# Zehong-Ma/MagCache

Measured on NVIDIA H100. Metric: denoising_steps_per_sec, higher is better.
Workload: dtype bf16

## Files before the change

### magcache_b200/csrc/attn_wgmma.cu

```cuda
#include <cstdlib>

#include "common.cuh"
#include "ptx.cuh"
#include "tma_host.cuh"

#ifndef MC_ATTN_EMU_DEFAULT
#define MC_ATTN_EMU_DEFAULT 0
#endif

namespace mc {

constexpr int kHD = 128;
constexpr int kLongMinLk = 1024;

struct AttnParams {
  int Lq, Lk, heads;
  int q_blocks, full_units, tail_units, tail_split;
  float* part_o;
  float2* part_ml;
  float scale_log2;
  __nv_bfloat16* out;
  int64_t ldo;
  int tile_rot;
  const uint32_t* seg_flags;
  const uint32_t* seg_epoch;
  int seg_rows;
};

struct WorkItem {
  int q_block, head;
  int split, nsplit;
  int tail_unit;
};

__device__ __forceinline__ WorkItem work_item(const AttnParams& p) {
  WorkItem w;
  int c = blockIdx.x, unit;
  if (c < p.full_units) {
    unit = c, w.split = 0, w.nsplit = 1, w.tail_unit = 0;
  } else {
    c -= p.full_units;
    w.tail_unit = c / p.tail_split;
    w.split = c - w.tail_unit * p.tail_split;
    w.nsplit = p.tail_split;
    unit = p.full_units + w.tail_unit;
  }
  w.head = unit / p.q_blocks;
  w.q_block = unit - w.head * p.q_blocks;
  return w;
}

template <uint32_t EMU_MASK>
__device__ __forceinline__ float exp2_sel(float x, int group) {
  return ((EMU_MASK >> (group & 7)) & 1u) ? ptx::ex2_emul(x) : ptx::ex2_approx(x);
}

__device__ __forceinline__ void wait_segments(const AttnParams& p, int row0, int rows) {
  if (p.seg_flags == nullptr) return;
  const uint32_t want = *reinterpret_cast<const volatile uint32_t*>(p.seg_epoch);
  const int last = min(row0 + rows, p.Lk) - 1;
  const int s0 = row0 / p.seg_rows, s1 = last / p.seg_rows;
  for (int s = s0; s <= s1; ++s) {
    const uint32_t* f = p.seg_flags + s;
    const long long t0 = clock64();
    for (;;) {
      uint32_t v;
      asm volatile("ld.acquire.sys.global.u32 %0, [%1];" : "=r"(v) : "l"(f) : "memory");
      if (static_cast<int32_t>(v - want) >= 0) break;
      __nanosleep(100);
      if (clock64() - t0 > MC_MBAR_TIMEOUT_CYCLES) {
        MC_DIAG("attention: key segment %d never arrived (flag %u, epoch %u)\n", s, v, want);
        __trap();
      }
    }
  }
  asm volatile("fence.proxy.async;" ::: "memory");
}

namespace ak {
constexpr int kBQ = 128;
constexpr int kQBytes = kBQ * kHD * 2;
constexpr int kThreads = 384;
constexpr int kProducerRegs = 24, kConsumerRegs = 240;
template <int BKV>
struct Layout {
  static constexpr int kKBytes = BKV * kHD * 2;
  static constexpr int kVBytes = BKV * kHD * 2;
  static constexpr int kOffK = kQBytes;
  static constexpr int kOffV = kOffK + 2 * kKBytes;
  static constexpr int kOffBar = kOffV + 2 * kVBytes;
  static constexpr int kSmem = kOffBar + 128;
};
}

template <int BKV, uint32_t EMU_MASK>
__global__ void __launch_bounds__(ak::kThreads, 1)
    attn_kernel(const __grid_constant__ CUtensorMap tmap_q, const __grid_constant__ CUtensorMap tmap_k,
                const __grid_constant__ CUtensorMap tmap_v, const AttnParams p) {
  using namespace ak;
  using L = Layout<BKV>;
  extern __shared__ __align__(1024) uint8_t smem[];
  uint64_t* bars = reinterpret_cast<uint64_t*>(smem + L::kOffBar);
  uint64_t* q_full = bars + 0;
  uint64_t* k_full = bars + 1;
  uint64_t* k_empty = bars + 3;
  uint64_t* v_full = bars + 5;
  uint64_t* v_empty = bars + 7;

  const int warp = threadIdx.x >> 5, lane = threadIdx.x & 31;
  const WorkItem wi = work_item(p);
  const int q0 = wi.q_block * kBQ;
  const int head = wi.head;
  const int total_tiles = (p.Lk + BKV - 1) / BKV;
  const int per_split = (total_tiles + wi.nsplit - 1) / wi.nsplit;
  const int t0 = wi.split * per_split;
  const int n_tiles = min(per_split, total_tiles - t0);
  auto tile_of = [&](int j) {
    int t = p.tile_rot + t0 + j;
    return t >= total_tiles ? t - total_tiles : t;
  };

  if (threadIdx.x == 0) {
    if ((ptx::smem_u32(smem) & 1023u) != 0) {
      MC_DIAG("attn_kernel: dynamic smem base not 1024-aligned\n");
      __trap();
    }
    ptx::prefetch_tmap(&tmap_q);
    ptx::prefetch_tmap(&tmap_k);
    ptx::prefetch_tmap(&tmap_v);
    ptx::mbar_init(q_full, 1);
    for (int s = 0; s < 2; ++s) {
      ptx::mbar_init(&k_full[s], 1);
      ptx::mbar_init(&k_empty[s], 8);
      ptx::mbar_init(&v_full[s], 1);
      ptx::mbar_init(&v_empty[s], 8);
    }
    ptx::fence_mbar_init();
  }
  __syncthreads();

  if (warp < 4) {
    ptx::setmaxnreg_dec<kProducerRegs>();
    if (warp == 0) {
      if (ptx::elect_one()) {
        ptx::mbar_expect_tx(q_full, kQBytes);
        ptx::tma_load_2d(smem, &tmap_q, q_full, head * kHD, q0);
        ptx::tma_load_2d(smem + kQBytes / 2, &tmap_q, q_full, head * kHD + 64, q0);
      }
      __syncwarp();
      for (int j = 0; j < n_tiles; ++j) {
        const int s = j & 1;
        const uint32_t ph = (j >> 1) & 1;
        const int kv0 = tile_of(j) * BKV;
        if (p.seg_flags != nullptr) {
          if (lane == 0) wait_segments(p, kv0, BKV);
          __syncwarp();
        }
        ptx::mbar_wait(&k_empty[s], ph ^ 1);
        if (ptx::elect_one()) {
          ptx::mbar_expect_tx(&k_full[s], L::kKBytes);
          ptx::tma_load_2d(smem + L::kOffK + s * L::kKBytes, &tmap_k, &k_full[s], head * kHD, kv0);
          ptx::tma_load_2d(smem + L::kOffK + s * L::kKBytes + L::kKBytes / 2, &tmap_k, &k_full[s], head * kHD + 64, kv0);
        }
        __syncwarp();
        ptx::mbar_wait(&v_empty[s], ph ^ 1);
        if (ptx::elect_one()) {
          ptx::mbar_expect_tx(&v_full[s], L::kVBytes);
          ptx::tma_load_2d(smem + L::kOffV + s * L::kVBytes, &tmap_v, &v_full[s], head * kHD, kv0);
          ptx::tma_load_2d(smem + L::kOffV + s * L::kVBytes + L::kVBytes / 2, &tmap_v, &v_full[s], head * kHD + 64, kv0);
        }
        __syncwarp();
      }
    }
  } else {
    ptx::setmaxnreg_inc<kConsumerRegs>();
    const int wg = (warp >> 2) - 1;
    const int r = wg * 64 + (warp & 3) * 16 + (lane >> 2);
    const int cq = 2 * (lane & 3);
    const uint32_t q_base = ptx::smem_u32(smem) + wg * (64 * 128);
    const uint32_t k_base = ptx::smem_u32(smem + L::kOffK), v_base = ptx::smem_u32(smem + L::kOffV);
    int j_ragged = -1;
    if (p.Lk % BKV != 0) {
      int jr = total_tiles - 1 - p.tile_rot - t0;
      if (jr < 0) jr += total_tiles;
      if (jr < n_tiles) j_ragged = jr;
    }
    float o[kHD / 2];
#pragma unroll
    for (int i = 0; i < kHD / 2; ++i) o[i] = 0.f;
    float m0 = -INFINITY, m1 = -INFINITY, l0 = 0.f, l1 = 0.f;
    bool timed_out = false;
    ptx::mbar_wait_or_flag(q_full, 0, timed_out);

    constexpr uint32_t kTurnThreads = 256;
    const uint32_t bar_own = 1 + wg, bar_other = 2 - wg;
    auto turn_begin = [&] { ptx::named_bar_sync(bar_own, kTurnThreads); };
    auto turn_end = [&] { ptx::named_bar_arrive(bar_other, kTurnThreads); };
    if (wg == 0) ptx::named_bar_arrive(bar_own, kTurnThreads);

    float sc[BKV / 2];
    uint32_t pa[BKV / 16][4];
    const int valid = p.Lk - (total_tiles - 1) * BKV;
    auto issue_s = [&](int j) {
      const int s = j & 1;
      ptx::wgmma_fence();
#pragma unroll
      for (int kk = 0; kk < kHD / 16; ++kk) {
        const uint64_t da = ptx::gmma_desc_sw128_kmajor(q_base + (kk >> 2) * (kQBytes / 2)) + 2 * (kk & 3);
        const uint64_t db = ptx::gmma_desc_sw128_kmajor(k_base + s * L::kKBytes + (kk >> 2) * (L::kKBytes / 2)) + 2 * (kk & 3);
        if constexpr (BKV == 128) {
          ptx::wgmma_m64n128k16_ss(sc, da, db, kk != 0 ? 1u : 0u);
        } else {
          ptx::wgmma_m64n64k16_ss(sc, da, db, kk != 0 ? 1u : 0u);
        }
      }
      ptx::wgmma_commit();
    };
    auto issue_pv = [&](int j) {
      const int s = j & 1;
      ptx::fence_regs(o);
      ptx::wgmma_fence();
      const uint64_t dv = ptx::gmma_desc_sw128_mnmajor(v_base + s * L::kVBytes, BKV * 128);
#pragma unroll
      for (int kk = 0; kk < BKV / 16; ++kk)
        ptx::wgmma_m64n128k16_rs_tb(o, pa[kk], dv + static_cast<uint64_t>(kk * (2048 / 16)), 1u);
      ptx::wgmma_commit();
    };
    auto softmax = [&](int j, float& f0, float& f1) {
      ptx::fence_regs(sc);
      __syncwarp();
      if (lane == 0) ptx::mbar_arrive(&k_empty[j & 1]);
      if (j == j_ragged) {
#pragma unroll
        for (int i = 0; i < BKV / 8; ++i)
#pragma unroll
          for (int e = 0; e < 4; ++e)
            if (8 * i + cq + (e & 1) >= valid) sc[4 * i + e] = -INFINITY;
      }
      float mx0 = -INFINITY, mx1 = -INFINITY;
#pragma unroll
      for (int i = 0; i < BKV / 8; ++i) {
        mx0 = fmaxf(mx0, fmaxf(sc[4 * i], sc[4 * i + 1]));
        mx1 = fmaxf(mx1, fmaxf(sc[4 * i + 2], sc[4 * i + 3]));
      }
#pragma unroll
      for (int off = 1; off <= 2; off <<= 1) {
        mx0 = fmaxf(mx0, __shfl_xor_sync(0xffffffffu, mx0, off));
        mx1 = fmaxf(mx1, __shfl_xor_sync(0xffffffffu, mx1, off));
      }
      const float mn0 = fmaxf(m0, mx0 * p.scale_log2), mn1 = fmaxf(m1, mx1 * p.scale_log2);
      f0 = ptx::ex2_approx(m0 - mn0), f1 = ptx::ex2_approx(m1 - mn1);
      m0 = mn0, m1 = mn1;
      l0 *= f0, l1 *= f1;
#pragma unroll
      for (int i = 0; i < BKV / 8; ++i) {
        sc[4 * i] = exp2_sel<EMU_MASK>(fmaf(sc[4 * i], p.scale_log2, -m0), i);
        sc[4 * i + 1] = exp2_sel<EMU_MASK>(fmaf(sc[4 * i + 1], p.scale_log2, -m0), i);
        sc[4 * i + 2] = exp2_sel<EMU_MASK>(fmaf(sc[4 * i + 2], p.scale_log2, -m1), i);
        sc[4 * i + 3] = exp2_sel<EMU_MASK>(fmaf(sc[4 * i + 3], p.scale_log2, -m1), i);
        l0 += sc[4 * i] + sc[4 * i + 1];
        l1 += sc[4 * i + 2] + sc[4 * i + 3];
      }
    };
    auto pack_p = [&] {
#pragma unroll
      for (int i = 0; i < BKV / 8; ++i) {
        pa[i >> 1][(i & 1) * 2] = pack_bf16x2(sc[4 * i], sc[4 * i + 1]);
        pa[i >> 1][(i & 1) * 2 + 1] = pack_bf16x2(sc[4 * i + 2], sc[4 * i + 3]);
      }
    };
    auto release_v = [&](int j) {
      ptx::fence_regs(o);
      __syncwarp();
      if (lane == 0) ptx::mbar_arrive(&v_empty[j & 1]);
    };
    auto rescale_o = [&](float f0, float f1) {
#pragma unroll
      for (int i = 0; i < kHD / 8; ++i) {
        o[4 * i] *= f0, o[4 * i + 1] *= f0;
        o[4 * i + 2] *= f1, o[4 * i + 3] *= f1;
      }
    };
    {
      ptx::mbar_wait_or_flag(&k_full[0], 0, timed_out);
      turn_begin();
      issue_s(0);
      turn_end();
      ptx::wgmma_wait<0>();
      float f0, f1;
      softmax(0, f0, f1);
      rescale_o(f0, f1);
      pack_p();
    }
    for (int j = 1; j < n_tiles; ++j) {
      ptx::mbar_wait_or_flag(&k_full[j & 1], (j >> 1) & 1, timed_out);
      ptx::mbar_wait_or_flag(&v_full[(j - 1) & 1], ((j - 1) >> 1) & 1, timed_out);
      turn_begin();
      issue_s(j);
      issue_pv(j - 1);
      turn_end();
      ptx::wgmma_wait<1>();
      float f0, f1;
      softmax(j, f0, f1);
      ptx::wgmma_wait<0>();
      release_v(j - 1);
      rescale_o(f0, f1);
      pack_p();
    }
    {
      const int j = n_tiles - 1;
      ptx::mbar_wait_or_flag(&v_full[j & 1], (j >> 1) & 1, timed_out);
      turn_begin();
      issue_pv(j);
      if (wg == 0) turn_end();
      ptx::wgmma_wait<0>();
      release_v(j);
    }
    if (timed_out) __trap();

#pragma unroll
    for (int off = 1; off <= 2; off <<= 1) {
      l0 += __shfl_xor_sync(0xffffffffu, l0, off);
      l1 += __shfl_xor_sync(0xffffffffu, l1, off);
    }
    const bool partial = wi.nsplit > 1;
#pragma unroll
    for (int h = 0; h < 2; ++h) {
      const float inv_l = 1.0f / (h ? l1 : l0);
      const int rt = r + 8 * h;
      const int row = q0 + rt;
      if (row >= p.Lq) continue;
      if (partial) {
        const int64_t prow = (static_cast<int64_t>(wi.split) * p.tail_units + wi.tail_unit) * kBQ + rt;
        if ((lane & 3) == 0) p.part_ml[prow] = make_float2(h ? m1 : m0, h ? l1 : l0);
        float* dst = p.part_o + prow * kHD + cq;
#pragma unroll
        for (int i = 0; i < kHD / 8; ++i)
          *reinterpret_cast<float2*>(dst + 8 * i) = make_float2(o[4 * i + 2 * h] * inv_l, o[4 * i + 2 * h + 1] * inv_l);
      } else {
        __nv_bfloat16* dst = p.out + static_cast<int64_t>(row) * p.ldo + head * kHD + cq;
#pragma unroll
        for (int i = 0; i < kHD / 8; ++i)
          *reinterpret_cast<uint32_t*>(dst + 8 * i) = pack_bf16x2(o[4 * i + 2 * h] * inv_l, o[4 * i + 2 * h + 1] * inv_l);
      }
    }
  }
}

__global__ void __launch_bounds__(256) attn_combine_kernel(const float* __restrict__ part_o, const float2* __restrict__ part_ml, int nsplit,
                                                           int tail_units, int full_units, int q_blocks, int rows_per_cta, int Lq,
                                                           __nv_bfloat16* __restrict__ out, int64_t ldo) {
  constexpr int kGroups = kHD / 8;
  const int64_t total = static_cast<int64_t>(tail_units) * rows_per_cta * kGroups;
  const int64_t split_stride = static_cast<int64_t>(tail_units) * rows_per_cta;
  for (int64_t i = static_cast<int64_t>(blockIdx.x) * blockDim.x + threadIdx.x; i < total; i += static_cast<int64_t>(gridDim.x) * blockDim.x) {
    const int64_t prow = i / kGroups;
    const int g = static_cast<int>(i - prow * kGroups);
    const int tu = static_cast<int>(prow / rows_per_cta), r = static_cast<int>(prow - static_cast<int64_t>(tu) * rows_per_cta);
    const int unit = full_units + tu;
    const int head = unit / q_blocks, row = (unit - head * q_blocks) * rows_per_cta + r;
    if (row >= Lq) continue;
    float mmax = -INFINITY;
    for (int s = 0; s < nsplit; ++s) mmax = fmaxf(mmax, part_ml[s * split_stride + prow].x);
    float acc[8] = {0.f, 0.f, 0.f, 0.f, 0.f, 0.f, 0.f, 0.f};
    float wsum = 0.f;
    for (int s = 0; s < nsplit; ++s) {
      const float2 ml = part_ml[s * split_stride + prow];
      const float w = ml.y * ptx::ex2_approx(ml.x - mmax);
      wsum += w;
      float v[8];
      ptx::ld_nc_v8_f32(part_o + (s * split_stride + prow) * kHD + g * 8, v);
#pragma unroll
      for (int j = 0; j < 8; ++j) acc[j] = fmaf(w, v[j], acc[j]);
    }
    const float inv = 1.0f / wsum;
#pragma unroll
    for (int j = 0; j < 8; ++j) acc[j] *= inv;
    *reinterpret_cast<uint4*>(out + static_cast<int64_t>(row) * ldo + head * kHD + g * 8) = pack_bf16x8(acc);
  }
}

struct AttnPlan {
  bool long_kernel;
  int q_blocks, kv_tile, total_tiles, rows_per_cta;
  int full_units, tail_units, tail_split;
  size_t ws_bytes;
  int grid() const { return full_units + tail_units * tail_split; }
};

static int env_int(const char* name, int lo, int hi, int dflt) {
  const char* e = getenv(name);
  if (!e || !*e) return dflt;
  const int v = atoi(e);
  return (v < lo || v > hi) ? dflt : v;
}

static AttnPlan plan_attention(int Lq, int Lk, int heads, bool need_long = false) {
  AttnPlan pl;
  const int forced_splits = env_int("MC_ATTN_SPLITS", 1, 16, 0);
  const int kernel_sel = env_int("MC_ATTN_KERNEL", 0, 2, 0);
  pl.long_kernel = need_long || kernel_sel == 2 || (kernel_sel == 0 && Lk >= kLongMinLk);
  pl.rows_per_cta = ak::kBQ;
  pl.kv_tile = pl.long_kernel ? 128 : 64;
  pl.q_blocks = (Lq + pl.rows_per_cta - 1) / pl.rows_per_cta;
  pl.total_tiles = (Lk + pl.kv_tile - 1) / pl.kv_tile;
  const int64_t units = static_cast<int64_t>(pl.q_blocks) * heads;
  const int slots = num_sms();
  const int min_tiles_per_split = pl.long_kernel ? 4 : 8;
  int full = static_cast<int>(units), tail = 0, split = 1;
  if (forced_splits > 0) {
    if (forced_splits > 1) full = 0, tail = static_cast<int>(units), split = forced_splits;
  } else {
    const int rem = static_cast<int>(units % slots);
    const int by_tiles = pl.total_tiles / min_tiles_per_split;
    int f = rem > 0 ? slots / rem : 1;
    if (f > 8) f = 8;
    if (f > by_tiles) f = by_tiles;
    if (f >= 2) full = static_cast<int>(units) - rem, tail = rem, split = f;
  }
  if (split > pl.total_tiles) split = pl.total_tiles;
  if (split > 1) {
    const int per = (pl.total_tiles + split - 1) / split;
    split = (pl.total_tiles + per - 1) / per;
  }
  if (split <= 1) full = static_cast<int>(units), tail = 0, split = 1;
  pl.full_units = full, pl.tail_units = tail, pl.tail_split = split;
  pl.ws_bytes = tail > 0 ? static_cast<size_t>(split) * tail * pl.rows_per_cta * (kHD * sizeof(float) + sizeof(float2)) : 0;
  return pl;
}

}

extern "C" int32_t mc_attn_workspace_bytes(int32_t Lq, int32_t Lk, int32_t heads, int64_t* bytes_out) {
  MC_CHECK_ARG(bytes_out != nullptr && Lq >= 1 && Lk >= 1 && heads >= 1, "mc_attn_workspace_bytes: bad arguments");
  const size_t a = mc::plan_attention(Lq, Lk, heads, false).ws_bytes, b = mc::plan_attention(Lq, Lk, heads, true).ws_bytes;
  *bytes_out = static_cast<int64_t>(a > b ? a : b);
  return MC_OK;
}

extern "C" int32_t mc_attn_fwd_ex(const void* q, int64_t ldq, const void* k, int64_t ldk, const void* v, int64_t ldv, void* out,
                                  int64_t ldo, int32_t Lq, int32_t Lk, int32_t heads, float scale, void* workspace,
                                  int64_t workspace_bytes, int32_t first_key_row, const uint32_t* seg_flags, const uint32_t* seg_epoch,
                                  int32_t seg_rows, void* stream) {
  MC_CHECK_ARG(q && k && v && out, "mc_attn_fwd: null pointer");
  MC_CHECK_ARG(Lq >= 1 && Lk >= 1 && heads >= 1, "mc_attn_fwd: Lq=%d Lk=%d heads=%d", Lq, Lk, heads);
  const int64_t width = static_cast<int64_t>(heads) * mc::kHD;
  MC_CHECK_ARG(ldq >= width && ldk >= width && ldo >= width && ldv >= width, "mc_attn_fwd: leading dimensions too small");
  MC_CHECK_ARG(ldq % 8 == 0 && ldk % 8 == 0 && ldv % 8 == 0 && ldo % 8 == 0, "mc_attn_fwd: leading dimensions must be multiples of 8");
  MC_CHECK_ARG(mc::aligned16(q) && mc::aligned16(k) && mc::aligned16(v) && mc::aligned16(out), "mc_attn_fwd: pointers must be 16-byte aligned");
  MC_CHECK_ARG(first_key_row >= 0 && first_key_row < Lk, "mc_attn_fwd: first_key_row=%d outside [0, %d)", first_key_row, Lk);
  MC_CHECK_ARG(seg_flags == nullptr || (seg_rows >= 1 && seg_epoch != nullptr), "mc_attn_fwd: seg_rows=%d / null epoch", seg_rows);
  const mc::AttnPlan pl = mc::plan_attention(Lq, Lk, heads, first_key_row != 0 || seg_flags != nullptr);
  MC_CHECK_ARG(static_cast<int64_t>(pl.q_blocks) * heads * 8 < INT32_MAX, "mc_attn_fwd: grid too large");
  if (pl.tail_units > 0) {
    MC_CHECK_ARG(workspace != nullptr && workspace_bytes >= static_cast<int64_t>(pl.ws_bytes) && (reinterpret_cast<uintptr_t>(workspace) & 31u) == 0,
                 "mc_attn_fwd: split-KV needs a 32-byte aligned workspace of %lld bytes (mc_attn_workspace_bytes), got %lld",
                 static_cast<long long>(pl.ws_bytes), static_cast<long long>(workspace_bytes));
  }
  const int q_box = mc::ak::kBQ;
  CUtensorMap tq, tk, tv;
  int32_t rc = mc::make_tmap_bf16_2d(&tq, q, static_cast<uint64_t>(Lq), static_cast<uint64_t>(width), static_cast<uint64_t>(ldq), q_box, 64);
  if (rc) return rc;
  rc = mc::make_tmap_bf16_2d(&tk, k, static_cast<uint64_t>(Lk), static_cast<uint64_t>(width), static_cast<uint64_t>(ldk), pl.kv_tile, 64);
  if (rc) return rc;
  rc = mc::make_tmap_bf16_2d(&tv, v, static_cast<uint64_t>(Lk), static_cast<uint64_t>(width), static_cast<uint64_t>(ldv), pl.kv_tile, 64);
  if (rc) return rc;

  float* part_o = static_cast<float*>(workspace);
  const size_t part_rows = static_cast<size_t>(pl.tail_split) * pl.tail_units * pl.rows_per_cta;
  float2* part_ml = pl.tail_units > 0 ? reinterpret_cast<float2*>(part_o + part_rows * mc::kHD) : nullptr;
  mc::AttnParams p{};
  p.Lq = Lq, p.Lk = Lk, p.heads = heads;
  p.q_blocks = pl.q_blocks, p.full_units = pl.full_units, p.tail_units = pl.tail_units, p.tail_split = pl.tail_split;
  p.part_o = pl.tail_units > 0 ? part_o : nullptr, p.part_ml = part_ml;
  p.scale_log2 = scale * 1.4426950408889634f;
  p.out = static_cast<__nv_bfloat16*>(out), p.ldo = ldo;
  p.tile_rot = ((first_key_row + pl.kv_tile - 1) / pl.kv_tile) % pl.total_tiles;
  p.seg_flags = seg_flags, p.seg_epoch = seg_epoch, p.seg_rows = seg_rows > 0 ? seg_rows : Lk;

  dim3 grid(pl.grid(), 1, 1);
  cudaStream_t st = static_cast<cudaStream_t>(stream);
  if (pl.long_kernel) {
    static mc::PerDeviceOnce once[4];
    const int emu = mc::env_int("MC_ATTN_EMU", 0, 4, MC_ATTN_EMU_DEFAULT);
#define MC_LAUNCH_LONG(MASK, IDX)                                                                                                    \
  do {                                                                                                                               \
    rc = mc::set_max_smem_once(mc::attn_kernel<128, MASK>, mc::ak::Layout<128>::kSmem, once[IDX], "cudaFuncSetAttribute(attn smem)"); \
    if (rc) return rc;                                                                                                               \
    mc::attn_kernel<128, MASK><<<grid, mc::ak::kThreads, mc::ak::Layout<128>::kSmem, st>>>(tq, tk, tv, p);                           \
  } while (0)
    switch (emu) {
      case 2: MC_LAUNCH_LONG(0x88u, 1); break;
      case 3: MC_LAUNCH_LONG(0x92u, 2); break;
      case 4: MC_LAUNCH_LONG(0xAAu, 3); break;
      default: MC_LAUNCH_LONG(0x00u, 0); break;
    }
#undef MC_LAUNCH_LONG
  } else {
    static mc::PerDeviceOnce once;
    rc = mc::set_max_smem_once(mc::attn_kernel<64, 0u>, mc::ak::Layout<64>::kSmem, once, "cudaFuncSetAttribute(attn smem)");
    if (rc) return rc;
    mc::attn_kernel<64, 0u><<<grid, mc::ak::kThreads, mc::ak::Layout<64>::kSmem, st>>>(tq, tk, tv, p);
  }
  MC_CHECK_LAUNCH("attn_kernel launch");
  if (pl.tail_units > 0) {
    const int64_t total = static_cast<int64_t>(pl.tail_units) * pl.rows_per_cta * (mc::kHD / 8);
    const int64_t want = (total + 255) / 256, cap = static_cast<int64_t>(mc::num_sms()) * 8;
    mc::attn_combine_kernel<<<static_cast<int>(want < cap ? want : cap), 256, 0, st>>>(
        p.part_o, p.part_ml, pl.tail_split, pl.tail_units, pl.full_units, pl.q_blocks, pl.rows_per_cta, Lq, static_cast<__nv_bfloat16*>(out), ldo);
    MC_CHECK_LAUNCH("attn_combine_kernel launch");
  }
  return MC_OK;
}

extern "C" int32_t mc_attn_fwd(const void* q, int64_t ldq, const void* k, int64_t ldk, const void* v, int64_t ldv, void* out,
                               int64_t ldo, int32_t Lq, int32_t Lk, int32_t heads, float scale, void* workspace,
                               int64_t workspace_bytes, void* stream) {
  return mc_attn_fwd_ex(q, ldq, k, ldk, v, ldv, out, ldo, Lq, Lk, heads, scale, workspace, workspace_bytes, 0, nullptr, nullptr, 0, stream);
}
```

Before: 1.660.

## Multicast K/V tiles across 2-CTA clusters in long attention kernel

For the long (BKV=128) attention kernel, CTAs are grouped into clusters of two that process adjacent query blocks of the same head. Each CTA loads half of every K/V tile and multicasts it to both CTAs, so each tile is read from L2 once per cluster instead of once per CTA. Empty-barrier release now arrives on both CTAs' barriers, work-item mapping and q_blocks are padded to cluster multiples, and slots are sized by the cluster occupancy query. The costs are cross-CTA coupling, where the slower CTA stalls its partner, possible padding of wasted query blocks, and a cluster sync at exit.

```diff
diff --git a/magcache_b200/csrc/attn_wgmma.cu b/magcache_b200/csrc/attn_wgmma.cu
--- a/magcache_b200/csrc/attn_wgmma.cu
+++ b/magcache_b200/csrc/attn_wgmma.cu
@@ -33,6 +33,7 @@
   int tail_unit;
 };
 
+template <int C>
 __device__ __forceinline__ WorkItem work_item(const AttnParams& p) {
   WorkItem w;
   int c = blockIdx.x, unit;
@@ -40,8 +41,9 @@
     unit = c, w.split = 0, w.nsplit = 1, w.tail_unit = 0;
   } else {
     c -= p.full_units;
-    w.tail_unit = c / p.tail_split;
-    w.split = c - w.tail_unit * p.tail_split;
+    const int cl = c / C, tail_cl = cl / p.tail_split;
+    w.split = cl - tail_cl * p.tail_split;
+    w.tail_unit = C * tail_cl + (c - cl * C);
     w.nsplit = p.tail_split;
     unit = p.full_units + w.tail_unit;
   }
@@ -78,19 +80,25 @@
 }
 
 namespace ak {
+template <int BKV>
+constexpr int kCluster = BKV == 128 ? 2 : 1;
+constexpr int kStages = 2;
 constexpr int kBQ = 128;
 constexpr int kQBytes = kBQ * kHD * 2;
 constexpr int kThreads = 384;
+constexpr int kConsumerWarps = 8;
 constexpr int kProducerRegs = 24, kConsumerRegs = 240;
 template <int BKV>
 struct Layout {
   static constexpr int kKBytes = BKV * kHD * 2;
   static constexpr int kVBytes = BKV * kHD * 2;
   static constexpr int kOffK = kQBytes;
-  static constexpr int kOffV = kOffK + 2 * kKBytes;
-  static constexpr int kOffBar = kOffV + 2 * kVBytes;
+  static constexpr int kOffV = kOffK + kStages * kKBytes;
+  static constexpr int kOffBar = kOffV + kStages * kVBytes;
   static constexpr int kSmem = kOffBar + 128;
 };
+__device__ __forceinline__ int stage(int j) { return static_cast<int>(static_cast<uint32_t>(j) % kStages); }
+__device__ __forceinline__ uint32_t phase(int j) { return (static_cast<uint32_t>(j) / kStages) & 1u; }
 }
 
 template <int BKV, uint32_t EMU_MASK>
@@ -99,16 +107,18 @@
                 const __grid_constant__ CUtensorMap tmap_v, const AttnParams p) {
   using namespace ak;
   using L = Layout<BKV>;
+  constexpr int C = kCluster<BKV>;
   extern __shared__ __align__(1024) uint8_t smem[];
   uint64_t* bars = reinterpret_cast<uint64_t*>(smem + L::kOffBar);
   uint64_t* q_full = bars + 0;
   uint64_t* k_full = bars + 1;
-  uint64_t* k_empty = bars + 3;
-  uint64_t* v_full = bars + 5;
-  uint64_t* v_empty = bars + 7;
+  uint64_t* k_empty = bars + 1 + kStages;
+  uint64_t* v_full = bars + 1 + 2 * kStages;
+  uint64_t* v_empty = bars + 1 + 3 * kStages;
 
   const int warp = threadIdx.x >> 5, lane = threadIdx.x & 31;
-  const WorkItem wi = work_item(p);
+  const uint32_t rank = C > 1 ? ptx::cluster_ctarank() : 0u;
+  const WorkItem wi = work_item<C>(p);
   const int q0 = wi.q_block * kBQ;
   const int head = wi.head;
   const int total_tiles = (p.Lk + BKV - 1) / BKV;
@@ -129,15 +139,20 @@
     ptx::prefetch_tmap(&tmap_k);
     ptx::prefetch_tmap(&tmap_v);
     ptx::mbar_init(q_full, 1);
-    for (int s = 0; s < 2; ++s) {
+    for (int s = 0; s < kStages; ++s) {
       ptx::mbar_init(&k_full[s], 1);
-      ptx::mbar_init(&k_empty[s], 8);
+      ptx::mbar_init(&k_empty[s], C * kConsumerWarps);
       ptx::mbar_init(&v_full[s], 1);
-      ptx::mbar_init(&v_empty[s], 8);
+      ptx::mbar_init(&v_empty[s], C * kConsumerWarps);
     }
     ptx::fence_mbar_init();
   }
-  __syncthreads();
+  if constexpr (C > 1) {
+    ptx::cluster_arrive();
+    ptx::cluster_wait();
+  } else {
+    __syncthreads();
+  }
 
   if (warp < 4) {
     ptx::setmaxnreg_dec<kProducerRegs>();
@@ -148,9 +163,19 @@
         ptx::tma_load_2d(smem + kQBytes / 2, &tmap_q, q_full, head * kHD + 64, q0);
       }
       __syncwarp();
+      constexpr uint16_t kAll = (1u << C) - 1;
+      const int col = head * kHD + static_cast<int>(rank) * 64;
+      auto load = [&](uint8_t* dst, const CUtensorMap* tmap, uint64_t* bar, int kv0) {
+        if constexpr (C > 1) {
+          ptx::tma_load_2d_multicast(dst + rank * (L::kKBytes / 2), tmap, bar, col, kv0, kAll);
+        } else {
+          ptx::tma_load_2d(dst, tmap, bar, head * kHD, kv0);
+          ptx::tma_load_2d(dst + L::kKBytes / 2, tmap, bar, head * kHD + 64, kv0);
+        }
+      };
       for (int j = 0; j < n_tiles; ++j) {
-        const int s = j & 1;
-        const uint32_t ph = (j >> 1) & 1;
+        const int s = stage(j);
+        const uint32_t ph = phase(j);
         const int kv0 = tile_of(j) * BKV;
         if (p.seg_flags != nullptr) {
           if (lane == 0) wait_segments(p, kv0, BKV);
@@ -159,15 +184,13 @@
         ptx::mbar_wait(&k_empty[s], ph ^ 1);
         if (ptx::elect_one()) {
           ptx::mbar_expect_tx(&k_full[s], L::kKBytes);
-          ptx::tma_load_2d(smem + L::kOffK + s * L::kKBytes, &tmap_k, &k_full[s], head * kHD, kv0);
-          ptx::tma_load_2d(smem + L::kOffK + s * L::kKBytes + L::kKBytes / 2, &tmap_k, &k_full[s], head * kHD + 64, kv0);
+          load(smem + L::kOffK + s * L::kKBytes, &tmap_k, &k_full[s], kv0);
         }
         __syncwarp();
         ptx::mbar_wait(&v_empty[s], ph ^ 1);
         if (ptx::elect_one()) {
           ptx::mbar_expect_tx(&v_full[s], L::kVBytes);
-          ptx::tma_load_2d(smem + L::kOffV + s * L::kVBytes, &tmap_v, &v_full[s], head * kHD, kv0);
-          ptx::tma_load_2d(smem + L::kOffV + s * L::kVBytes + L::kVBytes / 2, &tmap_v, &v_full[s], head * kHD + 64, kv0);
+          load(smem + L::kOffV + s * L::kVBytes, &tmap_v, &v_full[s], kv0);
         }
         __syncwarp();
       }
@@ -198,11 +221,21 @@
     auto turn_end = [&] { ptx::named_bar_arrive(bar_other, kTurnThreads); };
     if (wg == 0) ptx::named_bar_arrive(bar_own, kTurnThreads);
 
+    auto release = [&](uint64_t* bar) {
+      __syncwarp();
+      if (lane == 0) {
+        if constexpr (C > 1) {
+          for (uint32_t c = 0; c < C; ++c) ptx::mbar_arrive_cluster(bar, c);
+        } else {
+          ptx::mbar_arrive(bar);
+        }
+      }
+    };
     float sc[BKV / 2];
     uint32_t pa[BKV / 16][4];
     const int valid = p.Lk - (total_tiles - 1) * BKV;
     auto issue_s = [&](int j) {
-      const int s = j & 1;
+      const int s = stage(j);
       ptx::wgmma_fence();
 #pragma unroll
       for (int kk = 0; kk < kHD / 16; ++kk) {
@@ -217,7 +250,7 @@
       ptx::wgmma_commit();
     };
     auto issue_pv = [&](int j) {
-      const int s = j & 1;
+      const int s = stage(j);
       ptx::fence_regs(o);
       ptx::wgmma_fence();
       const uint64_t dv = ptx::gmma_desc_sw128_mnmajor(v_base + s * L::kVBytes, BKV * 128);
@@ -228,8 +261,7 @@
     };
     auto softmax = [&](int j, float& f0, float& f1) {
       ptx::fence_regs(sc);
-      __syncwarp();
-      if (lane == 0) ptx::mbar_arrive(&k_empty[j & 1]);
+      release(&k_empty[stage(j)]);
       if (j == j_ragged) {
 #pragma unroll
         for (int i = 0; i < BKV / 8; ++i)
@@ -271,8 +303,7 @@
     };
     auto release_v = [&](int j) {
       ptx::fence_regs(o);
-      __syncwarp();
-      if (lane == 0) ptx::mbar_arrive(&v_empty[j & 1]);
+      release(&v_empty[stage(j)]);
     };
     auto rescale_o = [&](float f0, float f1) {
 #pragma unroll
@@ -293,8 +324,8 @@
       pack_p();
     }
     for (int j = 1; j < n_tiles; ++j) {
-      ptx::mbar_wait_or_flag(&k_full[j & 1], (j >> 1) & 1, timed_out);
-      ptx::mbar_wait_or_flag(&v_full[(j - 1) & 1], ((j - 1) >> 1) & 1, timed_out);
+      ptx::mbar_wait_or_flag(&k_full[stage(j)], phase(j), timed_out);
+      ptx::mbar_wait_or_flag(&v_full[stage(j - 1)], phase(j - 1), timed_out);
       turn_begin();
       issue_s(j);
       issue_pv(j - 1);
@@ -309,7 +340,7 @@
     }
     {
       const int j = n_tiles - 1;
-      ptx::mbar_wait_or_flag(&v_full[j & 1], (j >> 1) & 1, timed_out);
+      ptx::mbar_wait_or_flag(&v_full[stage(j)], phase(j), timed_out);
       turn_begin();
       issue_pv(j);
       if (wg == 0) turn_end();
@@ -344,6 +375,10 @@
           *reinterpret_cast<uint32_t*>(dst + 8 * i) = pack_bf16x2(o[4 * i + 2 * h] * inv_l, o[4 * i + 2 * h + 1] * inv_l);
       }
     }
+  }
+  if constexpr (C > 1) {
+    ptx::cluster_arrive();
+    ptx::cluster_wait();
   }
 }
 
@@ -395,6 +430,42 @@
   return (v < lo || v > hi) ? dflt : v;
 }
 
+template <int BKV>
+struct AttnLaunch {
+  cudaLaunchAttribute attr[1];
+  cudaLaunchConfig_t cfg = {};
+  AttnLaunch(int grid, cudaStream_t st) {
+    attr[0].id = cudaLaunchAttributeClusterDimension;
+    attr[0].val.clusterDim.x = ak::kCluster<BKV>, attr[0].val.clusterDim.y = 1, attr[0].val.clusterDim.z = 1;
+    cfg.gridDim = dim3(grid, 1, 1);
+    cfg.blockDim = dim3(ak::kThreads, 1, 1);
+    cfg.dynamicSmemBytes = ak::Layout<BKV>::kSmem;
+    cfg.stream = st;
+    cfg.attrs = attr;
+    cfg.numAttrs = ak::kCluster<BKV> > 1 ? 1 : 0;
+  }
+};
+
+template <int BKV>
+static int attn_slots() {
+  constexpr int C = ak::kCluster<BKV>;
+  if (C == 1) return num_sms();
+  static int cached[kMaxDevices] = {};
+  const int d = current_device();
+  if (cached[d] > 0) return cached[d];
+  AttnLaunch<BKV> la(C * num_sms(), nullptr);
+  int n = 0;
+  if (cudaFuncSetAttribute(attn_kernel<BKV, 0u>, cudaFuncAttributeMaxDynamicSharedMemorySize, ak::Layout<BKV>::kSmem) != cudaSuccess ||
+      cudaOccupancyMaxActiveClusters(&n, attn_kernel<BKV, 0u>, &la.cfg) != cudaSuccess)
+    n = 0;
+  if (n < 1) {
+    (void)cudaGetLastError();
+    return num_sms() / C * C;
+  }
+  cached[d] = C * n;
+  return cached[d];
+}
+
 static AttnPlan plan_attention(int Lq, int Lk, int heads, bool need_long = false) {
   AttnPlan pl;
   const int forced_splits = env_int("MC_ATTN_SPLITS", 1, 16, 0);
@@ -402,10 +473,12 @@
   pl.long_kernel = need_long || kernel_sel == 2 || (kernel_sel == 0 && Lk >= kLongMinLk);
   pl.rows_per_cta = ak::kBQ;
   pl.kv_tile = pl.long_kernel ? 128 : 64;
+  const int cluster = pl.long_kernel ? ak::kCluster<128> : ak::kCluster<64>;
   pl.q_blocks = (Lq + pl.rows_per_cta - 1) / pl.rows_per_cta;
+  pl.q_blocks = (pl.q_blocks + cluster - 1) / cluster * cluster;
   pl.total_tiles = (Lk + pl.kv_tile - 1) / pl.kv_tile;
   const int64_t units = static_cast<int64_t>(pl.q_blocks) * heads;
-  const int slots = num_sms();
+  const int slots = pl.long_kernel ? attn_slots<128>() : attn_slots<64>();
   const int min_tiles_per_split = pl.long_kernel ? 4 : 8;
   int full = static_cast<int>(units), tail = 0, split = 1;
   if (forced_splits > 0) {
@@ -478,7 +551,7 @@
   p.tile_rot = ((first_key_row + pl.kv_tile - 1) / pl.kv_tile) % pl.total_tiles;
   p.seg_flags = seg_flags, p.seg_epoch = seg_epoch, p.seg_rows = seg_rows > 0 ? seg_rows : Lk;
 
-  dim3 grid(pl.grid(), 1, 1);
+  const int grid = pl.grid();
   cudaStream_t st = static_cast<cudaStream_t>(stream);
   if (pl.long_kernel) {
     static mc::PerDeviceOnce once[4];
@@ -487,7 +560,9 @@
   do {                                                                                                                               \
     rc = mc::set_max_smem_once(mc::attn_kernel<128, MASK>, mc::ak::Layout<128>::kSmem, once[IDX], "cudaFuncSetAttribute(attn smem)"); \
     if (rc) return rc;                                                                                                               \
-    mc::attn_kernel<128, MASK><<<grid, mc::ak::kThreads, mc::ak::Layout<128>::kSmem, st>>>(tq, tk, tv, p);                           \
+    const mc::AttnLaunch<128> la(grid, st);                                                                                          \
+    const cudaError_t e = cudaLaunchKernelEx(&la.cfg, mc::attn_kernel<128, MASK>, tq, tk, tv, p);                                    \
+    if (e != cudaSuccess) return mc::cuda_fail(e, "attn_kernel launch");                                                            \
   } while (0)
     switch (emu) {
       case 2: MC_LAUNCH_LONG(0x88u, 1); break;
```

New measurement: 1.688, median of 6. +1.7%, better.
